# luokn/ms-gat

Measured on AMD Instinct MI355X. Metric: MS-GAT fwd+bwd samples/sec (B×T node-updates/s), PEMSD7 N=883 T=12, higher is better.
Workload: dtype f32

## Files before the change

### ms_gat_amd/csrc/aggregate.hip

```cpp
#include "common.hpp"
#include "sell.hpp"

namespace msgat {


struct __attribute__((packed, aligned(4))) int4u { int v[4]; };
struct __attribute__((packed, aligned(4))) float4u { float v[4]; };

template <int T4, typename RowPtr>
__device__ __forceinline__ float4 gather_row(const int* __restrict__ idx, const float* __restrict__ Eg,
                                             int e0, int e1, int nnz, RowPtr rows, int j) {
  float4 acc = f4zero();
  if (nnz < 8) {
    for (int e = e0; e < e1; ++e) f4fma(Eg[e], rows[idx[e] * T4 + j], acc);
    return acc;
  }
  const int b0 = min(e0, nnz - 8);
  const int4u m0 = *reinterpret_cast<const int4u*>(idx + b0);
  const int4u m1 = *reinterpret_cast<const int4u*>(idx + b0 + 4);
  const float4u w0 = *reinterpret_cast<const float4u*>(Eg + b0);
  const float4u w1 = *reinterpret_cast<const float4u*>(Eg + b0 + 4);
#pragma unroll
  for (int k = 0; k < 4; ++k) {
    const float wa = (b0 + k >= e0 && b0 + k < e1) ? w0.v[k] : 0.f;
    const float wb = (b0 + 4 + k >= e0 && b0 + 4 + k < e1) ? w1.v[k] : 0.f;
    f4fma(wa, rows[m0.v[k] * T4 + j], acc);
    f4fma(wb, rows[m1.v[k] * T4 + j], acc);
  }
  for (int e = b0 + 8; e < e1; e += 4) {
    const int b = min(e, nnz - 4);
    const int4u m = *reinterpret_cast<const int4u*>(idx + b);
    const float4u w = *reinterpret_cast<const float4u*>(Eg + b);
#pragma unroll
    for (int k = 0; k < 4; ++k) {
      const float wk = (b + k >= e && b + k < e1) ? w.v[k] : 0.f;
      f4fma(wk, rows[m.v[k] * T4 + j], acc);
    }
  }
  return acc;
}

template <int T4, bool DOT>
__global__ __launch_bounds__(kAggBlock) void k_agg_lds(
    const int* __restrict__ ptr, const int* __restrict__ idx, const float4* __restrict__ u4,
    const float* __restrict__ E, const float* __restrict__ addvec,
    const float4* __restrict__ extra4, float4* __restrict__ v4, int Bg, int Cu, int N, int nnz,
    int CH, const float4* __restrict__ xdot4, float* __restrict__ dap) {
  extern __shared__ float4 slab[];
  __shared__ float dred[kAggBlock / 64][kAggDotMaxC];
  const int g = blockIdx.y;
  const int r = g / Bg;
  const int c0 = blockIdx.x * CH;
  const int ch = min(CH, Cu - c0);
  const int NT4 = N * T4;
  const size_t base = ((size_t)g * Cu + c0) * NT4;
  const int total = ch * NT4;

  for (int i = threadIdx.x; i < total; i += kAggBlock) slab[i] = u4[base + i];
  __syncthreads();

  const int seg = cdiv(NT4, (int)gridDim.z);
  const int s_end = min((int)(blockIdx.z + 1) * seg, NT4);
  float da[kAggDotMaxC] = {0.f, 0.f, 0.f, 0.f};
  const float* Eg = E + (size_t)g * nnz;
  for (int s = blockIdx.z * seg + threadIdx.x; s < s_end; s += kAggBlock) {
    const int n = s / T4;
    const int j = s - n * T4;
    const int e0 = ptr[n], e1 = ptr[n + 1];
    float4 ex = f4zero();
    if (addvec != nullptr) ex = extra4[(size_t)g * NT4 + s];
    if (DOT) {
#pragma unroll
      for (int c = 0; c < kAggDotMaxC; ++c)
        if (c < ch) da[c] = f4dot(ex, xdot4[base + (size_t)c * NT4 + s], da[c]);
    }
    for (int c = 0; c < ch; ++c) {
      float4 acc = gather_row<T4>(idx, Eg, e0, e1, nnz, slab + c * NT4, j);
      if (addvec != nullptr) f4fma(addvec[r * Cu + c0 + c], ex, acc);
      v4[base + (size_t)c * NT4 + s] = acc;
    }
  }
  if (DOT) {
    const int wave = threadIdx.x >> 6, lane = threadIdx.x & 63;
#pragma unroll
    for (int c = 0; c < kAggDotMaxC; ++c) {
      float w = da[c];
#pragma unroll
      for (int off = 32; off > 0; off >>= 1) w += __shfl_xor(w, off);
      if (lane == 0) dred[wave][c] = w;
    }
    __syncthreads();
    if (threadIdx.x < ch) {
      float t = 0.f;
#pragma unroll
      for (int w = 0; w < kAggBlock / 64; ++w) t += dred[w][threadIdx.x];
      dap[((size_t)g * gridDim.z + blockIdx.z) * Cu + c0 + threadIdx.x] = t;
    }
  }
}

#ifndef MSGAT_RING_AUX
#define MSGAT_RING_AUX 0
#endif
template <int T4, int KI>
__global__ __launch_bounds__(kAggBlock) void k_agg_ring(
    const int* __restrict__ ptr, const int* __restrict__ idx, const float4* __restrict__ u4,
    const float* __restrict__ E, float4* __restrict__ v4, int Cu, int N, int nnz, int nslab, int per) {
  typedef __attribute__((address_space(3))) void* lds_ptr_t;
  typedef const __attribute__((address_space(1))) void* glb_ptr_t;
  extern __shared__ float4 ring[];
  constexpr int kWaves = kAggBlock / 64;
  constexpr int kBufF4 = KI * kAggBlock;
  const int NT4 = N * T4;
  const int wave = __builtin_amdgcn_readfirstlane(threadIdx.x >> 6), lane = threadIdx.x & 63;
  const int s0 = blockIdx.x * per, ns = min(per, nslab - s0);
  if (ns <= 0) return;

  auto issue = [&](int t) {
    const float4* src = u4 + (size_t)(s0 + min(t, ns - 1)) * NT4;
    float4* buf = ring + (t % 3) * kBufF4;
#pragma unroll
    for (int k = 0; k < KI; ++k) {
      const int i0 = (wave + kWaves * k) * 64;
      __builtin_amdgcn_global_load_lds((glb_ptr_t)(src + min(i0 + lane, NT4 - 1)), (lds_ptr_t)(buf + i0), 16, 0, MSGAT_RING_AUX);
    }
  };

  issue(0);
  issue(1);

  int slot[KI], jof[KI], e0s[KI], e1s[KI], b0s[KI];
  int m[KI][8];
  float w[KI][8];
#pragma unroll
  for (int k = 0; k < KI; ++k) {
    slot[k] = min((int)threadIdx.x + kAggBlock * k, NT4 - 1);
    const int n = slot[k] / T4;
    jof[k] = slot[k] - n * T4;
    e0s[k] = ptr[n];
    e1s[k] = ptr[n + 1];
    b0s[k] = min(e0s[k], nnz - 8);
    const int4u ia = *reinterpret_cast<const int4u*>(idx + b0s[k]), ib = *reinterpret_cast<const int4u*>(idx + b0s[k] + 4);
#pragma unroll
    for (int q = 0; q < 4; ++q) {
      m[k][q] = (b0s[k] + q >= e0s[k] && b0s[k] + q < e1s[k]) ? ia.v[q] * T4 + jof[k] : jof[k];
      m[k][4 + q] = (b0s[k] + 4 + q >= e0s[k] && b0s[k] + 4 + q < e1s[k]) ? ib.v[q] * T4 + jof[k] : jof[k];
    }
  }
  auto load_weights = [&](int g) {
    const float* Eg = E + (size_t)g * nnz;
#pragma unroll
    for (int k = 0; k < KI; ++k) {
      const float4u wa = *reinterpret_cast<const float4u*>(Eg + b0s[k]), wb = *reinterpret_cast<const float4u*>(Eg + b0s[k] + 4);
#pragma unroll
      for (int q = 0; q < 4; ++q) {
        w[k][q] = (b0s[k] + q >= e0s[k] && b0s[k] + q < e1s[k]) ? wa.v[q] : 0.f;
        w[k][4 + q] = (b0s[k] + 4 + q >= e0s[k] && b0s[k] + 4 + q < e1s[k]) ? wb.v[q] : 0.f;
      }
    }
  };
  int gcur = s0 / Cu;
  load_weights(gcur);

  for (int t = 0; t < ns; ++t) {
    if (t == 0) wait_vmcnt<KI>();
    else if (t == 1) wait_vmcnt<2 * KI>();
    else wait_vmcnt<3 * KI>();
    lds_barrier();
    issue(t + 2);
    const int g = (s0 + t) / Cu;
    if (g != gcur) {
      gcur = g;
      load_weights(g);
    }
    const float4* buf = ring + (t % 3) * kBufF4;
    float4* out = v4 + (size_t)(s0 + t) * NT4;
    const float* Eg = E + (size_t)g * nnz;
#pragma unroll
    for (int k = 0; k < KI; ++k) {
      float4 acc = f4zero();
#pragma unroll
      for (int q = 0; q < 8; ++q) f4fma(w[k][q], buf[m[k][q]], acc);
      for (int e = b0s[k] + 8; e < e1s[k]; ++e) f4fma(Eg[e], buf[idx[e] * T4 + jof[k]], acc);
      out[slot[k]] = acc;
    }
  }
}

template <int T4>
__global__ __launch_bounds__(kAggBlock) void k_agg_cols(
    const int* __restrict__ ptr, const int* __restrict__ idx, const float4* __restrict__ u4,
    const float* __restrict__ E, const float* __restrict__ addvec,
    const float4* __restrict__ extra4, float4* __restrict__ v4, int Bg, int Cu, int N, int nnz) {
  extern __shared__ float4 slab[];
  const int g = blockIdx.y;
  const int r = g / Bg;
  const int c = blockIdx.x;
  const size_t base = ((size_t)g * Cu + c) * N * T4;
  const float* Eg = E + (size_t)g * nnz;
  const float av = (addvec != nullptr) ? addvec[r * Cu + c] : 0.f;
  for (int j = 0; j < T4; ++j) {
    for (int n = threadIdx.x; n < N; n += kAggBlock) slab[n] = u4[base + (size_t)n * T4 + j];
    __syncthreads();
    for (int n = threadIdx.x; n < N; n += kAggBlock) {
      float4 acc = gather_row<1>(idx, Eg, ptr[n], ptr[n + 1], nnz, slab, 0);
      if (addvec != nullptr) f4fma(av, extra4[((size_t)g * N + n) * T4 + j], acc);
      v4[base + (size_t)n * T4 + j] = acc;
    }
    __syncthreads();
  }
}

template <int T4>
__global__ __launch_bounds__(kAggBlock) void k_agg_sell(
    const int* __restrict__ slice_off, const int* __restrict__ lane_row, const uint16_t* __restrict__ sidx,
    const float4* __restrict__ u4, const float* __restrict__ Es, const float* __restrict__ addvec,
    const float4* __restrict__ extra4, float4* __restrict__ v4, int G, int Bg, int Cu, int N, int n_pos,
    int n_slices) {
  extern __shared__ float4 slab[];
  const int xcd = blockIdx.x & 7, slot = blockIdx.x >> 3;
  const int j = slot % T4;
  const int c = (slot / T4) % Cu;
  const int g = (slot / (T4 * Cu)) * 8 + xcd;
  if (g >= G) return;
  const int r = g / Bg;
  const int wave = __builtin_amdgcn_readfirstlane(threadIdx.x >> 6), lane = threadIdx.x & 63;
  const size_t base = ((size_t)g * Cu + c) * N * T4;
  const float* Eg = Es + (size_t)g * n_pos;
  const float av = (addvec != nullptr) ? addvec[r * Cu + c] : 0.f;
  stage_column<T4>(slab, u4 + base, j, N);
  __syncthreads();
  float4 accs[kSellMaxSlices];
#pragma unroll
  for (int i = 0; i < kSellMaxSlices; ++i) {
    accs[i] = f4zero();
    const int s = wave + i * (kAggBlock / 64);
    if (s < n_slices) {
      const int off = slice_off[s];
      const int ntrip = (slice_off[s + 1] - off) >> 8;
      const uint2* pi4 = reinterpret_cast<const uint2*>(sidx + off) + lane;
      const float4* pe4 = reinterpret_cast<const float4*>(Eg + off) + lane;
      float4 acc = f4zero();
      if (ntrip > 0) {
        SellTrip a, b, c4, d;
        sell_issue(pi4, pe4, 0, ntrip, a);
        sell_issue(pi4, pe4, 1, ntrip, b);
        sell_issue(pi4, pe4, 2, ntrip, c4);
        sell_issue(pi4, pe4, 3, ntrip, d);
        for (int t = 0; t < ntrip; t += kSD) {
          sell_gather(a, slab, acc);
          sell_issue(pi4, pe4, t + 4, ntrip, a);
          if (t + 1 < ntrip) sell_gather(b, slab, acc);
          sell_issue(pi4, pe4, t + 5, ntrip, b);
          if (t + 2 < ntrip) sell_gather(c4, slab, acc);
          sell_issue(pi4, pe4, t + 6, ntrip, c4);
          if (t + 3 < ntrip) sell_gather(d, slab, acc);
          sell_issue(pi4, pe4, t + 7, ntrip, d);
        }
      }
      accs[i] = acc;
    }
  }
  __syncthreads();
#pragma unroll
  for (int i = 0; i < kSellMaxSlices; ++i) {
    const int s = wave + i * (kAggBlock / 64);
    if (s < n_slices) {
      const int row = lane_row[64 * s + lane];
      if (row >= 0) slab[row] = accs[i];
    }
  }
  __syncthreads();
  for (int n = threadIdx.x; n < N; n += kAggBlock) {
    float4 acc = slab[n];
    if (addvec != nullptr) f4fma(av, extra4[((size_t)g * N + n) * T4 + j], acc);
    v4[base + (size_t)n * T4 + j] = acc;
  }
}


template <int T4>
__global__ __launch_bounds__(kBlock) void k_agg_glb(
    const int* __restrict__ ptr, const int* __restrict__ idx, const float4* __restrict__ u4,
    const float* __restrict__ E, const float* __restrict__ addvec,
    const float4* __restrict__ extra4, float4* __restrict__ v4, int Bg, int Cu, int N, int nnz) {
  const int g = blockIdx.z;
  const int r = g / Bg;
  const int c = blockIdx.y;
  const int NT4 = N * T4;
  const int s = blockIdx.x * kBlock + threadIdx.x;
  if (s >= NT4) return;
  const int n = s / T4;
  const int j = s - n * T4;
  const float4* sl = u4 + ((size_t)g * Cu + c) * NT4;
  float4 acc = gather_row<T4>(idx, E + (size_t)g * nnz, ptr[n], ptr[n + 1], nnz, sl, j);
  if (addvec != nullptr) f4fma(addvec[r * Cu + c], extra4[(size_t)g * NT4 + s], acc);
  v4[((size_t)g * Cu + c) * NT4 + s] = acc;
}

template <int T4>
static int launch_aggregate_t(const int* ptr, const int* idx, int nnz, const msgat_sell_t* sell, const float* u,
                              const float* E, const float* addvec, const float* extra, float* v, int G, int Bg,
                              int Cu, int N, hipStream_t s, const float* xdot, float* dap, int* dot_done) {
  const int T = 4 * T4;
  const int CH = slab_channels(N, T, Cu, kLdsBudget);
  if (sell != nullptr) {
    const size_t lds = (size_t)N * sizeof(float4);
    static LdsGrant granted;
    if (int st = grant_dynamic_lds(&k_agg_sell<T4>, lds, granted)) return st;
    hipLaunchKernelGGL((k_agg_sell<T4>), dim3((unsigned)cdiv(G, 8) * 8 * Cu * T4), dim3(kAggBlock), lds, s,
                       sell->slice_off, sell->lane_row, sell->idx, (const float4*)u, E, addvec, (const float4*)extra,
                       (float4*)v, G, Bg, Cu, N, sell->n_pos, sell->n_slices);
  } else if (addvec == nullptr && xdot == nullptr && nnz >= 8 && N * T4 <= 3 * kAggBlock && G * Cu >= 512) {
    const int ncu = device_cu_count();
    const int nslab = G * Cu, per = cdiv(nslab, ncu), nb = cdiv(nslab, per);
    const int KI = cdiv(N * T4, kAggBlock);
    const size_t lds = (size_t)3 * KI * kAggBlock * sizeof(float4);
#define MSGAT_RING(ki)                                                                                            \
    {                                                                                                               \
      static LdsGrant granted;                                                                                      \
      if (int st = grant_dynamic_lds(&k_agg_ring<T4, ki>, lds, granted)) return st;                                 \
      hipLaunchKernelGGL((k_agg_ring<T4, ki>), dim3(nb), dim3(kAggBlock), lds, s, ptr, idx, (const float4*)u, E,    \
                         (float4*)v, Cu, N, nnz, nslab, per);                                                       \
    }
    if (KI == 1) MSGAT_RING(1) else if (KI == 2) MSGAT_RING(2) else MSGAT_RING(3)
#undef MSGAT_RING
  } else if (CH >= 1) {
    const size_t lds = (size_t)CH * N * T * sizeof(float);
    static LdsGrant granted_plain, granted_dot;
    if (int st = grant_dynamic_lds(&k_agg_lds<T4, false>, lds, granted_plain)) return st;
    if (int st = grant_dynamic_lds(&k_agg_lds<T4, true>, lds, granted_dot)) return st;
    const int nblocks = cdiv(Cu, CH) * G;
    int split = device_cu_count() / max(nblocks, 1);
    split = max(1, min(min(split, kAggMaxSplit), (N * T4) / 256));
    dim3 grid(cdiv(Cu, CH), G, split);
    if (xdot != nullptr && dap != nullptr && addvec != nullptr && Cu <= kAggDotMaxC) {
      hipLaunchKernelGGL((k_agg_lds<T4, true>), grid, dim3(kAggBlock), lds, s, ptr, idx, (const float4*)u, E, addvec,
                         (const float4*)extra, (float4*)v, Bg, Cu, N, nnz, CH, (const float4*)xdot, dap);
      if (dot_done != nullptr) *dot_done = split;
    } else {
      hipLaunchKernelGGL((k_agg_lds<T4, false>), grid, dim3(kAggBlock), lds, s, ptr, idx, (const float4*)u, E, addvec,
                         (const float4*)extra, (float4*)v, Bg, Cu, N, nnz, CH, nullptr, nullptr);
    }
  } else if ((size_t)N * sizeof(float4) <= (size_t)kLdsMax - 1024 && nnz >= 8) {
    const size_t lds = (size_t)N * sizeof(float4);
    static LdsGrant granted;
    if (int st = grant_dynamic_lds(&k_agg_cols<T4>, lds, granted)) return st;
    hipLaunchKernelGGL(k_agg_cols<T4>, dim3(Cu, G), dim3(kAggBlock), lds, s, ptr, idx, (const float4*)u, E,
                       addvec, (const float4*)extra, (float4*)v, Bg, Cu, N, nnz);
  } else {
    dim3 grid(cdiv(N * T4, kBlock), Cu, G);
    hipLaunchKernelGGL(k_agg_glb<T4>, grid, dim3(kBlock), 0, s, ptr, idx, (const float4*)u, E, addvec,
                       (const float4*)extra, (float4*)v, Bg, Cu, N, nnz);
  }
  MSGAT_CHECK_LAUNCH();
  return MSGAT_OK;
}

int launch_aggregate(const int* ptr, const int* idx, int nnz, const msgat_sell_t* sell, const float* u,
                     const float* E, const float* addvec, const float* extra, float* v, int G, int Bg, int Cu,
                     int N, int T, hipStream_t s, const float* xdot, float* dap, int* dot_done) {
  if (dot_done != nullptr) *dot_done = 0;
  switch (T) {
    case 4: return launch_aggregate_t<1>(ptr, idx, nnz, sell, u, E, addvec, extra, v, G, Bg, Cu, N, s, xdot, dap, dot_done);
    case 8: return launch_aggregate_t<2>(ptr, idx, nnz, sell, u, E, addvec, extra, v, G, Bg, Cu, N, s, xdot, dap, dot_done);
    case 12: return launch_aggregate_t<3>(ptr, idx, nnz, sell, u, E, addvec, extra, v, G, Bg, Cu, N, s, xdot, dap, dot_done);
    case 16: return launch_aggregate_t<4>(ptr, idx, nnz, sell, u, E, addvec, extra, v, G, Bg, Cu, N, s, xdot, dap, dot_done);
  }
  return MSGAT_ERR_UNSUPPORTED;
}

__global__ __launch_bounds__(kBlock) void k_permute_edges(const float* __restrict__ E,
                                                          const int* __restrict__ perm,
                                                          float* __restrict__ Eo, int nnz, int n) {
  const int g = blockIdx.y;
  const int k = blockIdx.x * kBlock + threadIdx.x;
  if (k >= n) return;
  const int e = perm[k];
  Eo[(size_t)g * n + k] = (e >= 0) ? E[(size_t)g * nnz + e] : 0.f;
}

int launch_permute_edges(const float* E, const int* perm, float* Eo, int G, int nnz, int n, hipStream_t s) {
  if (n == 0) return MSGAT_OK;
  dim3 grid(cdiv(n, kBlock), G);
  hipLaunchKernelGGL(k_permute_edges, grid, dim3(kBlock), 0, s, E, perm, Eo, nnz, n);
  MSGAT_CHECK_LAUNCH();
  return MSGAT_OK;
}

template <int T4, int OT>
__global__ __launch_bounds__(kBlock) void k_agg_proj(
    const int* __restrict__ rowptr, const int* __restrict__ col, const float4* __restrict__ x4,
    const float* __restrict__ E, const float* __restrict__ W, float4* __restrict__ y4,
    float4* __restrict__ z4, int Bg, int C, int Co, int N, int nnz) {
  extern __shared__ float Wl[];
  const int g = blockIdx.y;
  const int r = g / Bg;
  const int o0 = blockIdx.z * OT;
  for (int i = threadIdx.x; i < C * OT; i += kBlock) {
    const int c = i / OT, oo = i - c * OT, o = o0 + oo;
    Wl[i] = (o < Co) ? W[((size_t)r * Co + o) * C + c] : 0.f;
  }
  __syncthreads();
  const int NT4 = N * T4;
  const int s = blockIdx.x * kBlock + threadIdx.x;
  if (s >= NT4) return;
  const int n = s / T4;
  const int j = s - n * T4;
  const float* Eg = E + (size_t)g * nnz;
  const int e0 = rowptr[n], e1 = rowptr[n + 1];

  float4 acc[OT];
#pragma unroll
  for (int oo = 0; oo < OT; ++oo) acc[oo] = f4zero();
  for (int c = 0; c < C; ++c) {
    const float4* sl = x4 + ((size_t)g * C + c) * NT4;
    float4 y = gather_row<T4>(col, Eg, e0, e1, nnz, sl, j);
    if (y4 != nullptr && blockIdx.z == 0) y4[((size_t)g * C + c) * NT4 + s] = y;
    const float4* wrow = reinterpret_cast<const float4*>(Wl + c * OT);
#pragma unroll
    for (int o4 = 0; o4 < OT / 4; ++o4) {
      const float4 w = wrow[o4];
      f4fma(w.x, y, acc[4 * o4 + 0]);
      f4fma(w.y, y, acc[4 * o4 + 1]);
      f4fma(w.z, y, acc[4 * o4 + 2]);
      f4fma(w.w, y, acc[4 * o4 + 3]);
    }
  }
#pragma unroll
  for (int oo = 0; oo < OT; ++oo) {
    const int o = o0 + oo;
    if (o < Co) z4[((size_t)g * Co + o) * NT4 + s] = acc[oo];
  }
}

template <int T4, int OT>
static int launch_agg_proj_t(const msgat_graph_t& gr, const float* x, const float* E, const float* W,
                             float* y, float* z, int G, int Bg, int C, int Co, int N,
                             hipStream_t s) {
  dim3 grid(cdiv(N * T4, kBlock), G, cdiv(Co, OT));
  const size_t lds = (size_t)C * OT * sizeof(float);
  hipLaunchKernelGGL((k_agg_proj<T4, OT>), grid, dim3(kBlock), lds, s, gr.rowptr, gr.col,
                     (const float4*)x, E, W, (float4*)y, (float4*)z, Bg, C, Co, N, gr.nnz);
  MSGAT_CHECK_LAUNCH();
  return MSGAT_OK;
}

template <int T4>
static int launch_agg_proj_o(const msgat_graph_t& gr, const float* x, const float* E, const float* W,
                             float* y, float* z, int G, int Bg, int C, int Co, int N,
                             hipStream_t s) {
  if (Co % 24 == 0) return launch_agg_proj_t<T4, 24>(gr, x, E, W, y, z, G, Bg, C, Co, N, s);
  if (Co % 32 == 0) return launch_agg_proj_t<T4, 32>(gr, x, E, W, y, z, G, Bg, C, Co, N, s);
  if (Co % 16 == 0) return launch_agg_proj_t<T4, 16>(gr, x, E, W, y, z, G, Bg, C, Co, N, s);
  if (Co <= 4) return launch_agg_proj_t<T4, 4>(gr, x, E, W, y, z, G, Bg, C, Co, N, s);
  return launch_agg_proj_t<T4, 8>(gr, x, E, W, y, z, G, Bg, C, Co, N, s);
}

int launch_aggregate_project(const msgat_graph_t& gr, const float* x, const float* E,
                             const float* W, float* y, float* z, int G, int Bg, int C, int Co,
                             int N, int T, hipStream_t s) {
  switch (T) {
    case 4: return launch_agg_proj_o<1>(gr, x, E, W, y, z, G, Bg, C, Co, N, s);
    case 8: return launch_agg_proj_o<2>(gr, x, E, W, y, z, G, Bg, C, Co, N, s);
    case 12: return launch_agg_proj_o<3>(gr, x, E, W, y, z, G, Bg, C, Co, N, s);
    case 16: return launch_agg_proj_o<4>(gr, x, E, W, y, z, G, Bg, C, Co, N, s);
  }
  return MSGAT_ERR_UNSUPPORTED;
}

template <int T4, bool USE_LDS>
__global__ __launch_bounds__(kBlock) void k_sddmm(
    const int* __restrict__ erow, const int* __restrict__ col, const float4* __restrict__ u4,
    const float4* __restrict__ dv4, float* __restrict__ dEp, int Cu, int N, int nnz, int CH,
    int nchunks) {
  extern __shared__ float4 slab[];
  const int g = blockIdx.z;
  const int k = blockIdx.y;
  const int c0 = k * CH;
  const int ch = min(CH, Cu - c0);
  const int NT4 = N * T4;
  const size_t base = ((size_t)g * Cu + c0) * NT4;
  if (USE_LDS) {
    const int total = ch * NT4;
    for (int i = threadIdx.x; i < total; i += kBlock) slab[i] = u4[base + i];
    __syncthreads();
  }
  float* out = dEp + ((size_t)g * nchunks + k) * nnz;
  for (int e = blockIdx.x * kBlock + threadIdx.x; e < nnz; e += gridDim.x * kBlock) {
    const int n = erow[e], m = col[e];
    float acc = 0.f;
    for (int c = 0; c < ch; ++c) {
      const float4* a = dv4 + base + (size_t)c * NT4 + (size_t)n * T4;
      const float4* b = USE_LDS ? (slab + c * NT4 + m * T4) : (u4 + base + (size_t)c * NT4 + (size_t)m * T4);
#pragma unroll
      for (int j = 0; j < T4; ++j) acc = f4dot(a[j], b[j], acc);
    }
    out[e] = acc;
  }
}

template <int T4, bool FIRST>
__device__ __forceinline__ float4 gather_row_dot(const int* __restrict__ idx, const float* __restrict__ Eg, int e0,
                                                 int e1, int nnz, const float4* rows, int j, const float4& own,
                                                 float* __restrict__ pd, int dummy) {
  float4 acc = f4zero();
  auto edge = [&](int k, bool valid, float w, const float4& r) {
    f4fma(valid ? w : 0.f, r, acc);
    const float d = f4dot(r, own, 0.f);
    const int a = valid ? k * T4 + j : dummy;
    pd[a] = FIRST ? d : pd[a] + d;
  };
  const int b0 = min(e0, nnz - 8);
  const int4u m0 = *reinterpret_cast<const int4u*>(idx + b0);
  const int4u m1 = *reinterpret_cast<const int4u*>(idx + b0 + 4);
  const float4u w0 = *reinterpret_cast<const float4u*>(Eg + b0);
  const float4u w1 = *reinterpret_cast<const float4u*>(Eg + b0 + 4);
  {
    float4 ra[4];
#pragma unroll
    for (int k = 0; k < 4; ++k) ra[k] = rows[m0.v[k] * T4 + j];
#pragma unroll
    for (int k = 0; k < 4; ++k) edge(b0 + k, b0 + k >= e0 && b0 + k < e1, w0.v[k], ra[k]);
  }
  __builtin_amdgcn_sched_barrier(0);
  {
    float4 rb[4];
#pragma unroll
    for (int k = 0; k < 4; ++k) rb[k] = rows[m1.v[k] * T4 + j];
#pragma unroll
    for (int k = 0; k < 4; ++k) edge(b0 + 4 + k, b0 + 4 + k >= e0 && b0 + 4 + k < e1, w1.v[k], rb[k]);
  }
  for (int e = b0 + 8; e < e1; e += 4) {
    const int b = min(e, nnz - 4);
    const int4u m = *reinterpret_cast<const int4u*>(idx + b);
    const float4u w = *reinterpret_cast<const float4u*>(Eg + b);
#pragma unroll
    for (int k = 0; k < 4; ++k) edge(b + k, b + k >= e && b + k < e1, w.v[k], rows[m.v[k] * T4 + j]);
  }
  return acc;
}

constexpr int kAgsBlock = 768;

template <int T4>
__global__ __launch_bounds__(kAgsBlock) void k_agg_sddmm(
    const int* __restrict__ ptr, const int* __restrict__ idx, const float4* __restrict__ dv4,
    const float* __restrict__ Ec, const float4* __restrict__ u4, float4* __restrict__ du4,
    float* __restrict__ dEp, int Cu, int N, int nnz, int CH, int nchunks, int dvgs) {
  extern __shared__ float4 slab[];
  const int g = blockIdx.y;
  const int kc = blockIdx.x;
  const int c0 = kc * CH;
  const int ch = min(CH, Cu - c0);
  const int NT4 = N * T4;
  const size_t base = ((size_t)g * Cu + c0) * NT4;
  const int total = ch * NT4;
  float* pd = reinterpret_cast<float*>(slab + CH * NT4);
  const int dummy = nnz * T4 + threadIdx.x;

  const size_t vbase = ((size_t)g * dvgs + c0) * NT4;
  for (int i = threadIdx.x; i < total; i += kAgsBlock) slab[i] = dv4[vbase + i];
  __syncthreads();

  const float* Eg = Ec + (size_t)g * nnz;
  for (int s = threadIdx.x; s < NT4; s += kAgsBlock) {
    const int n = s / T4;
    const int j = s - n * T4;
    const int e0 = ptr[n], e1 = ptr[n + 1];
    du4[base + s] = gather_row_dot<T4, true>(idx, Eg, e0, e1, nnz, slab, j, u4[base + s], pd, dummy);
    for (int c = 1; c < ch; ++c) {
      const float4 own = u4[base + (size_t)c * NT4 + s];
      du4[base + (size_t)c * NT4 + s] = gather_row_dot<T4, false>(idx, Eg, e0, e1, nnz, slab + c * NT4, j, own, pd, dummy);
    }
  }
  __syncthreads();
  float* out = dEp + ((size_t)g * nchunks + kc) * nnz;
  for (int k = threadIdx.x; k < nnz; k += kAgsBlock) {
    float a = pd[k * T4];
#pragma unroll
    for (int j = 1; j < T4; ++j) a += pd[k * T4 + j];
    out[k] = a;
  }
}

static size_t agg_sddmm_lds(int N, int T, int Cu, int nnz) {
  const int CH = slab_channels(N, T, Cu, kLdsBudget);
  return (size_t)CH * N * T * sizeof(float) + ((size_t)nnz * (T / 4) + kAgsBlock) * sizeof(float);
}

bool agg_sddmm_fusable(const msgat_graph_t& gr, int N, int T, int Cu) {
  if (gr.nnz < 8 || sell_usable(gr.sell_rows, gr.nnz, N, T) || sell_usable(gr.sell_cols, gr.nnz, N, T)) return false;
  if (slab_channels(N, T, Cu, kLdsBudget) < 1) return false;
  return agg_sddmm_lds(N, T, Cu, gr.nnz) <= (size_t)(kLdsMax / 2);
}

template <int T4>
static int launch_agg_sddmm_t(const msgat_graph_t& gr, const float* dv, const float* Ec, const float* u, float* du,
                              float* dEp, int G, int Cu, int N, hipStream_t s, int dvgs) {
  const int T = 4 * T4;
  const int CH = slab_channels(N, T, Cu, kLdsBudget);
  const size_t lds = agg_sddmm_lds(N, T, Cu, gr.nnz);
  {
    static LdsGrant granted;
    if (int st = grant_dynamic_lds(&k_agg_sddmm<T4>, lds, granted)) return st;
  }
  const int nchunks = cdiv(Cu, CH);
  hipLaunchKernelGGL(k_agg_sddmm<T4>, dim3(nchunks, G), dim3(kAgsBlock), lds, s, gr.colptr, gr.crow, (const float4*)dv,
                     Ec, (const float4*)u, (float4*)du, dEp, Cu, N, gr.nnz, CH, nchunks, dvgs > 0 ? dvgs : Cu);
  MSGAT_CHECK_LAUNCH();
  return MSGAT_OK;
}

int launch_agg_sddmm(const msgat_graph_t& gr, const float* dv, const float* Ec, const float* u, float* du, float* dEp,
                     int G, int Cu, int N, int T, hipStream_t s, int dvgs) {
  switch (T) {
    case 4: return launch_agg_sddmm_t<1>(gr, dv, Ec, u, du, dEp, G, Cu, N, s, dvgs);
    case 8: return launch_agg_sddmm_t<2>(gr, dv, Ec, u, du, dEp, G, Cu, N, s, dvgs);
    case 12: return launch_agg_sddmm_t<3>(gr, dv, Ec, u, du, dEp, G, Cu, N, s, dvgs);
    case 16: return launch_agg_sddmm_t<4>(gr, dv, Ec, u, du, dEp, G, Cu, N, s, dvgs);
  }
  return MSGAT_ERR_UNSUPPORTED;
}

template <int T4>
__global__ __launch_bounds__(kAggBlock) void k_sddmm_sell(
    const int* __restrict__ slice_off, const int* __restrict__ lane_row, const uint16_t* __restrict__ sidx,
    const float4* __restrict__ u4, const float4* __restrict__ dv4, float* dEp, int Cu, int N, int n_pos,
    int n_slices, int CH, int nchunks) {
  extern __shared__ float4 slab[];
  const int g = blockIdx.y;
  const int kc = blockIdx.x;
  const int c0 = kc * CH;
  const int ch = min(CH, Cu - c0);
  const int wave = __builtin_amdgcn_readfirstlane(threadIdx.x >> 6), lane = threadIdx.x & 63;
  float* out = dEp + ((size_t)g * nchunks + kc) * n_pos;
  for (int pass = 0; pass < ch * T4; ++pass) {
    const int c = pass / T4, j = pass - c * T4;
    const size_t base = ((size_t)g * Cu + c0 + c) * N * T4;
    stage_column<T4>(slab, u4 + base, j, N);
    __syncthreads();
    for (int s = wave; s < n_slices; s += kAggBlock / 64) {
      const int off = slice_off[s];
      const int ntrip = (slice_off[s + 1] - off) >> 8;
      if (ntrip == 0) continue;
      const int row = lane_row[64 * s + lane];
      const uint2* pi4 = reinterpret_cast<const uint2*>(sidx + off) + lane;
      float4* po4 = reinterpret_cast<float4*>(out + off) + lane;
      const float4 a = dv4[base + (size_t)max(row, 0) * T4 + j];
      auto finish = [&](const SellTrip& x, int t) {
        const int4 id = sell_unpack(x.id);
        float4 o;
        o.x = f4dot(a, slab[id.x], pass == 0 ? 0.f : x.e.x);
        o.y = f4dot(a, slab[id.y], pass == 0 ? 0.f : x.e.y);
        o.z = f4dot(a, slab[id.z], pass == 0 ? 0.f : x.e.z);
        o.w = f4dot(a, slab[id.w], pass == 0 ? 0.f : x.e.w);
        po4[64 * t] = o;
      };
      SellTrip ta, tb;
      sell_issue(pi4, po4, 0, ntrip, ta);
      for (int t = 0; t < ntrip; t += 2) {
        sell_issue(pi4, po4, t + 1, ntrip, tb);
        finish(ta, t);
        sell_issue(pi4, po4, t + 2, ntrip, ta);
        if (t + 1 < ntrip) finish(tb, t + 1);
      }
    }
    __syncthreads();
  }
}

constexpr int kRegTrips = 12;

template <int T4>
__global__ __launch_bounds__(kAggBlock) void k_sddmm_sellreg(
    const int* __restrict__ slice_off, const int* __restrict__ lane_row, const uint16_t* __restrict__ sidx,
    const float4* __restrict__ u4, const float4* __restrict__ dv4, float* __restrict__ dE, int G, int Cu, int N,
    int n_pos, int n_slices, int Q) {
  extern __shared__ float4 slab[];
  const int xcd = blockIdx.x & 7, slot = blockIdx.x >> 3;
  const int q = slot % Q;
  const int g = (slot / Q) * 8 + xcd;
  if (g >= G) return;
  const int wave = __builtin_amdgcn_readfirstlane(threadIdx.x >> 6), lane = threadIdx.x & 63;
  const int W = q * (kAggBlock / 64) + wave;
  const int sA = W, sB = n_slices - 1 - W;
  const bool hasA = sA < n_slices && sA <= sB, hasB = hasA && sB > sA;
  const int sAc = hasA ? sA : 0, sBc = hasB ? sB : 0;
  const int offA = slice_off[sAc], offB = slice_off[sBc];
  const int ntA = hasA ? (slice_off[sAc + 1] - offA) >> 8 : 0;
  const int ntB = hasB ? (slice_off[sBc + 1] - offB) >> 8 : 0;
  const int nt = ntA + ntB;
  const int rowA = max(lane_row[64 * sAc + lane], 0), rowB = max(lane_row[64 * sBc + lane], 0);

  const uint2* piA = reinterpret_cast<const uint2*>(sidx + offA) + lane;
  const uint2* piB = reinterpret_cast<const uint2*>(sidx + offB) + lane;
  uint2 ids[kRegTrips];
  float4 acc[kRegTrips];
#pragma unroll
  for (int t = 0; t < kRegTrips; ++t) {
    const int tt = min(t, max(nt - 1, 0));
    const uint2* p = (tt < ntA) ? piA + 64 * tt : piB + 64 * (tt - ntA);
    ids[t] = (nt > 0) ? *p : make_uint2(0u, 0u);
    acc[t] = f4zero();
  }

  for (int pass = 0; pass < Cu * T4; ++pass) {
    const int c = pass / T4, jr = pass - c * T4;
    const int j = (jr + q) % T4;
    const size_t base = ((size_t)g * Cu + c) * N * T4;
    const float4 aA = dv4[base + (size_t)rowA * T4 + j];
    const float4 aB = dv4[base + (size_t)rowB * T4 + j];
    stage_column<T4, 4>(slab, u4 + base, j, N);
    __syncthreads();
#pragma unroll
    for (int t = 0; t < kRegTrips; ++t) {
      if (t < nt) {
        const bool inA = t < ntA;
        const float4 a = make_float4(inA ? aA.x : aB.x, inA ? aA.y : aB.y, inA ? aA.z : aB.z, inA ? aA.w : aB.w);
        const int4 id = sell_unpack(ids[t]);
        acc[t].x = f4dot(a, slab[id.x], acc[t].x);
        acc[t].y = f4dot(a, slab[id.y], acc[t].y);
        acc[t].z = f4dot(a, slab[id.z], acc[t].z);
        acc[t].w = f4dot(a, slab[id.w], acc[t].w);
      }
    }
    __syncthreads();
  }

  float* out = dE + (size_t)g * n_pos;
  float4* poA = reinterpret_cast<float4*>(out + offA) + lane;
  float4* poB = reinterpret_cast<float4*>(out + offB) + lane;
#pragma unroll
  for (int t = 0; t < kRegTrips; ++t)
    if (t < nt) *((t < ntA) ? poA + 64 * t : poB + 64 * (t - ntA)) = acc[t];
}

static bool sddmm_in_registers(const msgat_sell_t& sl) { return sl.pair_trips > 0 && sl.pair_trips <= kRegTrips; }

int sddmm_chunks(int G, int Cu, int N, int T, const msgat_sell_t* sell) {
  if (sell != nullptr) {
    if (sddmm_in_registers(*sell)) return 1;
    const int want = max(1, min(Cu, cdiv(256, max(G, 1))));
    return cdiv(Cu, cdiv(Cu, want));
  }
  const int CH = slab_channels(N, T, Cu, kLdsBudget);
  return CH >= 1 ? cdiv(Cu, CH) : 1;
}

template <int T4>
static int launch_sddmm_t(const msgat_graph_t& gr, const float* u, const float* dv, float* dEp,
                          int G, int Cu, int N, hipStream_t s) {
  const int T = 4 * T4;
  const int CH = slab_channels(N, T, Cu, kLdsBudget);
  if (sell_usable(gr.sell_rows, gr.nnz, N, T)) {
    const msgat_sell_t& sl = gr.sell_rows;
    const int nch = sddmm_chunks(G, Cu, N, T, &sl);
    const int chj = cdiv(Cu, nch);
    const size_t lds = (size_t)N * sizeof(float4);
    if (sddmm_in_registers(sl)) {
      {
        static LdsGrant granted;
        if (int st = grant_dynamic_lds(&k_sddmm_sellreg<T4>, lds, granted)) return st;
      }
      const int Q = cdiv(sl.n_slices, 2 * (kAggBlock / 64));
      hipLaunchKernelGGL(k_sddmm_sellreg<T4>, dim3((unsigned)cdiv(G, 8) * 8 * Q), dim3(kAggBlock), lds, s, sl.slice_off,
                         sl.lane_row, sl.idx, (const float4*)u, (const float4*)dv, dEp, G, Cu, N, sl.n_pos, sl.n_slices, Q);
      MSGAT_CHECK_LAUNCH();
      return MSGAT_OK;
    }
    {
      static LdsGrant granted;
      if (int st = grant_dynamic_lds(&k_sddmm_sell<T4>, lds, granted)) return st;
    }
    hipLaunchKernelGGL(k_sddmm_sell<T4>, dim3(nch, G), dim3(kAggBlock), lds, s, sl.slice_off, sl.lane_row, sl.idx,
                       (const float4*)u, (const float4*)dv, dEp, Cu, N, sl.n_pos, sl.n_slices, chj, nch);
  } else if (CH >= 1) {
    const size_t lds = (size_t)CH * N * T * sizeof(float);
    {
      static LdsGrant granted;
      if (int st = grant_dynamic_lds(&k_sddmm<T4, true>, lds, granted)) return st;
    }
    const int nchunks = cdiv(Cu, CH);
    dim3 grid(1, nchunks, G);
    hipLaunchKernelGGL((k_sddmm<T4, true>), grid, dim3(kBlock), lds, s, gr.erow, gr.col,
                       (const float4*)u, (const float4*)dv, dEp, Cu, N, gr.nnz, CH, nchunks);
  } else {
    dim3 grid(min(cdiv(gr.nnz, kBlock), 1024), 1, G);
    hipLaunchKernelGGL((k_sddmm<T4, false>), grid, dim3(kBlock), 0, s, gr.erow, gr.col,
                       (const float4*)u, (const float4*)dv, dEp, Cu, N, gr.nnz, Cu, 1);
  }
  MSGAT_CHECK_LAUNCH();
  return MSGAT_OK;
}

int launch_sddmm(const msgat_graph_t& gr, const float* u, const float* dv, float* dEp, int G,
                 int Cu, int N, int T, hipStream_t s) {
  if (gr.nnz == 0) return MSGAT_OK;
  switch (T) {
    case 4: return launch_sddmm_t<1>(gr, u, dv, dEp, G, Cu, N, s);
    case 8: return launch_sddmm_t<2>(gr, u, dv, dEp, G, Cu, N, s);
    case 12: return launch_sddmm_t<3>(gr, u, dv, dEp, G, Cu, N, s);
    case 16: return launch_sddmm_t<4>(gr, u, dv, dEp, G, Cu, N, s);
  }
  return MSGAT_ERR_UNSUPPORTED;
}

}
```

Baseline: 47470.

## Software-pipeline colptr, edge-window and own loads across the agg-SDDMM row loop

The fused aggregate-SDDMM kernel now loads the CSR row pointers, the first edge window and the own-row value for its first rows before the LDS staging barrier, and prefetches the next row's pointers and own value while the current row is processed. The dv slab fill for the first few block-strides goes through registers, so those loads overlap the edge-metadata loads. The gather loop is generalised to a configurable group size between schedule barriers, and the edge-window load is hoisted into a struct. The intent is to hide global-memory latency of the index and pointer loads, at the cost of more register pressure and dropping __restrict__ on several inputs.

```diff
diff --git a/ms_gat_amd/csrc/aggregate.hip b/ms_gat_amd/csrc/aggregate.hip
--- a/ms_gat_amd/csrc/aggregate.hip
+++ b/ms_gat_amd/csrc/aggregate.hip
@@ -500,9 +500,29 @@
   }
 }
 
+
+struct EdgeWindow {
+  int b0;
+  int4u m0, m1;
+  float4u w0, w1;
+};
+__device__ __forceinline__ EdgeWindow load_edge_window(const int* __restrict__ idx, const float* __restrict__ Eg,
+                                                       int e0, int nnz) {
+  EdgeWindow w;
+  w.b0 = min(e0, nnz - 8);
+  w.m0 = *reinterpret_cast<const int4u*>(idx + w.b0);
+  w.m1 = *reinterpret_cast<const int4u*>(idx + w.b0 + 4);
+  w.w0 = *reinterpret_cast<const float4u*>(Eg + w.b0);
+  w.w1 = *reinterpret_cast<const float4u*>(Eg + w.b0 + 4);
+  return w;
+}
+
+constexpr int kAgsRows = 4;
+
 template <int T4, bool FIRST>
-__device__ __forceinline__ float4 gather_row_dot(const int* __restrict__ idx, const float* __restrict__ Eg, int e0,
-                                                 int e1, int nnz, const float4* rows, int j, const float4& own,
+__device__ __forceinline__ float4 gather_row_dot(const EdgeWindow& win, const int* __restrict__ idx,
+                                                 const float* __restrict__ Eg, int e0, int e1, int nnz,
+                                                 const float4* rows, int j, const float4& own,
                                                  float* __restrict__ pd, int dummy) {
   float4 acc = f4zero();
   auto edge = [&](int k, bool valid, float w, const float4& r) {
@@ -511,25 +531,18 @@
     const int a = valid ? k * T4 + j : dummy;
     pd[a] = FIRST ? d : pd[a] + d;
   };
-  const int b0 = min(e0, nnz - 8);
-  const int4u m0 = *reinterpret_cast<const int4u*>(idx + b0);
-  const int4u m1 = *reinterpret_cast<const int4u*>(idx + b0 + 4);
-  const float4u w0 = *reinterpret_cast<const float4u*>(Eg + b0);
-  const float4u w1 = *reinterpret_cast<const float4u*>(Eg + b0 + 4);
-  {
-    float4 ra[4];
-#pragma unroll
-    for (int k = 0; k < 4; ++k) ra[k] = rows[m0.v[k] * T4 + j];
-#pragma unroll
-    for (int k = 0; k < 4; ++k) edge(b0 + k, b0 + k >= e0 && b0 + k < e1, w0.v[k], ra[k]);
-  }
-  __builtin_amdgcn_sched_barrier(0);
-  {
-    float4 rb[4];
-#pragma unroll
-    for (int k = 0; k < 4; ++k) rb[k] = rows[m1.v[k] * T4 + j];
-#pragma unroll
-    for (int k = 0; k < 4; ++k) edge(b0 + 4 + k, b0 + 4 + k >= e0 && b0 + 4 + k < e1, w1.v[k], rb[k]);
+  const int b0 = win.b0;
+  const int4u &m0 = win.m0, &m1 = win.m1;
+  const float4u &w0 = win.w0, &w1 = win.w1;
+#pragma unroll
+  for (int h = 0; h < 8; h += kAgsRows) {
+    float4 r[kAgsRows];
+#pragma unroll
+    for (int k = 0; k < kAgsRows; ++k) r[k] = rows[(h + k < 4 ? m0.v[(h + k) & 3] : m1.v[(h + k) & 3]) * T4 + j];
+#pragma unroll
+    for (int k = 0; k < kAgsRows; ++k)
+      edge(b0 + h + k, b0 + h + k >= e0 && b0 + h + k < e1, h + k < 4 ? w0.v[(h + k) & 3] : w1.v[(h + k) & 3], r[k]);
+    __builtin_amdgcn_sched_barrier(0);
   }
   for (int e = b0 + 8; e < e1; e += 4) {
     const int b = min(e, nnz - 4);
@@ -542,11 +555,12 @@
 }
 
 constexpr int kAgsBlock = 768;
+constexpr int kAgsAhead = 4;
 
 template <int T4>
 __global__ __launch_bounds__(kAgsBlock) void k_agg_sddmm(
-    const int* __restrict__ ptr, const int* __restrict__ idx, const float4* __restrict__ dv4,
-    const float* __restrict__ Ec, const float4* __restrict__ u4, float4* __restrict__ du4,
+    const int* ptr, const int* idx, const float4* dv4,
+    const float* Ec, const float4* u4, float4* __restrict__ du4,
     float* __restrict__ dEp, int Cu, int N, int nnz, int CH, int nchunks, int dvgs) {
   extern __shared__ float4 slab[];
   const int g = blockIdx.y;
@@ -560,18 +574,56 @@
   const int dummy = nnz * T4 + threadIdx.x;
 
   const size_t vbase = ((size_t)g * dvgs + c0) * NT4;
-  for (int i = threadIdx.x; i < total; i += kAgsBlock) slab[i] = dv4[vbase + i];
+  const float* Eg = Ec + (size_t)g * nnz;
+  const int tid = threadIdx.x;
+  auto colptr_pair = [&](int s, int& a, int& b) {
+    const int n = min(s, NT4 - 1) / T4;
+    a = ptr[n];
+    b = ptr[n + 1];
+  };
+  int e0, e1, f0, f1;
+  colptr_pair(tid, e0, e1);
+  colptr_pair(tid + kAgsBlock, f0, f1);
+  for (int i = tid + kAgsAhead * kAgsBlock; i < total; i += kAgsBlock) slab[i] = dv4[vbase + i];
+  float4 stage[kAgsAhead];
+#pragma unroll
+  for (int k = 0; k < kAgsAhead; ++k) stage[k] = dv4[vbase + min(tid + k * kAgsBlock, total - 1)];
+  float4 own = u4[base + min(tid, NT4 - 1)];
+  EdgeWindow win = load_edge_window(idx, Eg, e0, nnz);
+#pragma unroll
+  for (int k = 0; k < kAgsAhead; ++k) slab[min(tid + k * kAgsBlock, total - 1)] = stage[k];
   __syncthreads();
 
-  const float* Eg = Ec + (size_t)g * nnz;
-  for (int s = threadIdx.x; s < NT4; s += kAgsBlock) {
+  float4 nown = own;
+#pragma unroll
+  for (int k = 0; k < kAgsAhead; ++k) {
+    const int s = tid + k * kAgsBlock;
+    if (s >= NT4) break;
+    const int n = s / T4;
+    const int j = s - n * T4;
+    if (k > 0) {
+      win = load_edge_window(idx, Eg, e0, nnz);
+      own = nown;
+      if (k + 1 < kAgsAhead) colptr_pair(s + kAgsBlock, f0, f1);
+    }
+    if (k + 1 < kAgsAhead) nown = u4[base + min(s + kAgsBlock, NT4 - 1)];
+    du4[base + s] = gather_row_dot<T4, true>(win, idx, Eg, e0, e1, nnz, slab, j, own, pd, dummy);
+    for (int c = 1; c < ch; ++c) {
+      const float4 ownc = u4[base + (size_t)c * NT4 + s];
+      const EdgeWindow wc = load_edge_window(idx, Eg, e0, nnz);
+      du4[base + (size_t)c * NT4 + s] = gather_row_dot<T4, false>(wc, idx, Eg, e0, e1, nnz, slab + c * NT4, j, ownc, pd, dummy);
+    }
+    e0 = f0, e1 = f1;
+  }
+  for (int s = tid + kAgsAhead * kAgsBlock; s < NT4; s += kAgsBlock) {
     const int n = s / T4;
     const int j = s - n * T4;
     const int e0 = ptr[n], e1 = ptr[n + 1];
-    du4[base + s] = gather_row_dot<T4, true>(idx, Eg, e0, e1, nnz, slab, j, u4[base + s], pd, dummy);
+    const EdgeWindow w = load_edge_window(idx, Eg, e0, nnz);
+    du4[base + s] = gather_row_dot<T4, true>(w, idx, Eg, e0, e1, nnz, slab, j, u4[base + s], pd, dummy);
     for (int c = 1; c < ch; ++c) {
-      const float4 own = u4[base + (size_t)c * NT4 + s];
-      du4[base + (size_t)c * NT4 + s] = gather_row_dot<T4, false>(idx, Eg, e0, e1, nnz, slab + c * NT4, j, own, pd, dummy);
+      const float4 ownc = u4[base + (size_t)c * NT4 + s];
+      du4[base + (size_t)c * NT4 + s] = gather_row_dot<T4, false>(w, idx, Eg, e0, e1, nnz, slab + c * NT4, j, ownc, pd, dummy);
     }
   }
   __syncthreads();
```

After: 47980, median of 6. 1.01x the previous value.
